# kr-colab/locator

Hardware: AMD Instinct MI355X
Metric: training samples/sec on 1000x100k-SNP matrix (higher is better)
Workload: dtype f32; 1 GPU; synthetic 1000 ind x 100000 SNPs uint8 (BASELINE.json configs[2]), single model fit per GPU, batch 32, 810 train / 90 validation; width=256, nlayers=10, graph=True, chained_steps=True, epochs_in_flight=2, replicates_per_gpu=1, replicates=single model, full=False

## Files before the change

locator_amd/csrc/stack_fused.hip:

```cpp
#include <stdlib.h>

#include <type_traits>

#include "common.h"
#include "stack_tail.h"

#ifndef SF_THREADS
#define SF_THREADS 512
#endif


__device__ __forceinline__ float sf_sumsq_train(float e0, float e1) {
#pragma clang fp contract(off)
    const float a = e0 * e0, b = e1 * e1;
    return b + a;
}
__device__ __forceinline__ float sf_sumsq_eval(float e0, float e1) { return fmaf(e1, e1, e0 * e0); }

template <int NHT, int R, bool TRAIN>
__global__ __launch_bounds__(SF_THREADS) void stack_fused_kernel(
    const float* __restrict__ a1_in, const float* __restrict__ Wh, const float* __restrict__ WhT,
    const float* __restrict__ bh, const float* __restrict__ wa, const float* __restrict__ ba,
    const float* __restrict__ wb, const float* __restrict__ bb, const uint8_t* __restrict__ mask, float keep_scale,
    int L, int n_pre, int n_b, const int32_t* __restrict__ rows, const float* __restrict__ Y,
    float* __restrict__ acts, float* __restrict__ adrop, float* __restrict__ dz, float* __restrict__ head_out,
    float* __restrict__ yhat, float* __restrict__ dist, int xcd_stride, int n_work, int slot_rows,
    const float* __restrict__ rd_partial, int rd_G, int64_t rd_MH, const float* __restrict__ rd_cvec8,
    const float* __restrict__ rd_b1) {
    constexpr int Hp = NHT * 32;
    constexpr int C4 = Hp / 4;
    constexpr int KG = SF_THREADS / C4;
    constexpr int KPG = Hp / KG;
    static_assert(SF_THREADS % C4 == 0 && Hp % KG == 0 && KPG >= 1, "unsupported width for the fused stack");
    __shared__ __attribute__((aligned(16))) float act[R][Hp];
    __shared__ __attribute__((aligned(16))) float part[KG][R][Hp];
    __shared__ float hs[R][8];

    if (xcd_stride > 1 && (blockIdx.x % xcd_stride) != 0) return;
    const int li = xcd_stride > 1 ? blockIdx.x / xcd_stride : blockIdx.x;
    if (li >= n_work) {
        const int n_x = xcd_stride > 1 ? 8 / xcd_stride : 1;
        const int nh_all = (int)(gridDim.x / (xcd_stride > 1 ? xcd_stride : 1)) - n_work;
        const int hid = (li - n_work) / n_x, nh = nh_all / n_x > 0 ? nh_all / n_x : 1;
        const int64_t n4 = (int64_t)(L - 1) * Hp * Hp / 4;
        const f32x4* w4 = reinterpret_cast<const f32x4*>(Wh);
        f32x4 sink = {0.f, 0.f, 0.f, 0.f};
        for (int64_t i = (int64_t)hid * SF_THREADS + threadIdx.x; i < n4; i += (int64_t)nh * SF_THREADS) {
            f32x4 v = w4[i];
            sink[0] += v[0];
        }
        if (TRAIN && WhT != nullptr) {
            const f32x4* t4 = reinterpret_cast<const f32x4*>(WhT);
            for (int64_t i = n4 - 1 - ((int64_t)hid * SF_THREADS + threadIdx.x); i >= 0; i -= (int64_t)nh * SF_THREADS) {
                f32x4 v = t4[i];
                sink[1] += v[0];
            }
        }
        asm volatile("" ::"v"(sink[0]), "v"(sink[1]));
        return;
    }
    const int t = threadIdx.x, c4 = t % C4, kq = t / C4;
    const int r0 = li * R;
    const int64_t blk = (int64_t)slot_rows * Hp, HH = (int64_t)Hp * Hp;

    constexpr int RING = KPG < 32 ? KPG : 32;
    constexpr int RW = RING >= 16 ? RING / 8 : 1;
    constexpr int NS = RING / RW, NTRIP = KPG / RING;
    constexpr int ROWB = C4 * 16;
    static_assert(KPG >= 2 && NS >= 2 && NS * RW == RING && NTRIP * RING == KPG, "a pass must be whole trips round the ring");
    static_assert(ROWB <= 4096 && (RW == 1 || 4096 % ROWB == 0), "row offsets are split into a register part and an immediate");
    constexpr int NO = (R * Hp + SF_THREADS - 1) / SF_THREADS;
    static_assert((R * Hp) % SF_THREADS == 0 || R * Hp < SF_THREADS, "epilogue slots");
    f32x4 ring[RING];
    constexpr int NOFF = (RW * ROWB + 4095) / 4096;
    uint32_t toff[NOFF];
#pragma unroll
    for (int n = 0; n < NOFF; ++n) toff[n] = ((uint32_t)(kq * KPG) * C4 + c4) * 16u + 4096u * n;
    auto load_slot = [&](const float* __restrict__ Wsrc, int c, int s) {
        const char* base = reinterpret_cast<const char*>(Wsrc) + (size_t)c * (RW * ROWB);
        static_assert(RW == 1 || RW == 4, "rows per slot");
        gload16_uniform<0>(ring[s * RW], base, toff[0]);
        if constexpr (RW == 4) {
            gload16_uniform<ROWB % 4096>(ring[s * RW + 1], base, toff[ROWB / 4096]);
            gload16_uniform<(2 * ROWB) % 4096>(ring[s * RW + 2], base, toff[2 * ROWB / 4096]);
            gload16_uniform<(3 * ROWB) % 4096>(ring[s * RW + 3], base, toff[3 * ROWB / 4096]);
        }
    };
    auto fma_slot = [&](int c, int s, f32x4 (&acc)[R]) {
#pragma unroll
        for (int j = 0; j < RW; ++j) {
#pragma unroll
            for (int r = 0; r < R; ++r) {
                const float a = act[r][kq * KPG + c * RW + j];
                acc[r][0] = fmaf(a, ring[s * RW + j][0], acc[r][0]);
                acc[r][1] = fmaf(a, ring[s * RW + j][1], acc[r][1]);
                acc[r][2] = fmaf(a, ring[s * RW + j][2], acc[r][2]);
                acc[r][3] = fmaf(a, ring[s * RW + j][3], acc[r][3]);
            }
        }
    };
    auto trip = [&](auto last, int c0, const float* __restrict__ Wn, int cn, f32x4 (&acc)[R]) {
        constexpr int N = (NS - 1) * RW + (decltype(last)::value ? NO : 0);
#pragma unroll
        for (int s = 0; s < NS; ++s) {
            if constexpr (RW == 4) vm_wait_slot<N>(ring[s * RW], ring[s * RW + 1], ring[s * RW + 2], ring[s * RW + 3]);
            else vm_wait_slot<N>(ring[s * RW]);
            fma_slot(c0 + s, s, acc);
#pragma unroll
            for (int r = 0; r < R; ++r) vm_landed(acc[r]);
            load_slot(Wn, cn + s, s);
        }
    };
    auto contract = [&](const float* __restrict__ Wcur, const float* __restrict__ Wnext, auto operands) {
        f32x4 acc[R];
#pragma unroll
        for (int r = 0; r < R; ++r) acc[r] = f32x4{0.f, 0.f, 0.f, 0.f};
#pragma unroll 1
        for (int tr = 0; tr + 1 < NTRIP; ++tr) trip(std::false_type{}, tr * NS, Wcur, (tr + 1) * NS, acc);
        operands();
        trip(std::true_type{}, (NTRIP - 1) * NS, Wnext, 0, acc);
#pragma unroll
        for (int r = 0; r < R; ++r) *reinterpret_cast<f32x4*>(&part[kq][r][4 * c4]) = acc[r];
    };
    auto ring_end = [&]() {
        vm_wait<0>();
#pragma unroll
        for (int k = 0; k < RING; ++k) vm_landed(ring[k]);
    };
    const int n_pass = TRAIN ? 2 * (L - 1) : (L - 1);
    auto wseq = [&](int p) -> const float* {
        if (p >= n_pass) return uniform_ptr(Wh);
        return uniform_ptr(p < L - 1 ? Wh + (int64_t)p * HH : WhT + (int64_t)(2 * (L - 1) - 1 - p) * HH);
    };
    auto ring_start = [&]() {
        const float* W0 = wseq(0);
#pragma unroll
        for (int s = 0; s < NS; ++s) load_slot(W0, s, s);
    };
    auto reduced = [&](int r, int n) {
        float s = 0.f;
#pragma unroll
        for (int g = 0; g < KG; ++g) s += part[g][r][n];
        return s;
    };

    static_assert(SF_THREADS % Hp == 0, "one pair of wa per thread needs a thread count that is a multiple of the width");
    float h_wa0 = 0.f, h_wa1 = 0.f;
    float h_ba0 = 0.f, h_ba1 = 0.f, h_w00 = 0.f, h_w01 = 0.f, h_w10 = 0.f, h_w11 = 0.f, h_bb0 = 0.f, h_bb1 = 0.f;
    float h_y0 = 0.f, h_y1 = 0.f;
    const bool has_y = Y != nullptr && t < R && r0 + t < n_b;

    if (!TRAIN && rd_partial != nullptr) {
        const int gq = (rd_G + 3) / 4;
        for (int i = t; i < R * Hp; i += SF_THREADS) {
            const int r = i / Hp, n = i % Hp;
            float v = 0.f;
            if (r0 + r < n_b) {
                const float* src = rd_partial + (int64_t)(r0 + r) * Hp + n;
                float sq[4];
#pragma unroll
                for (int q = 0; q < 4; ++q) {
                    const int g0 = q * gq, g1 = g0 + gq < rd_G ? g0 + gq : rd_G;
                    float z = 0.f;
                    for (int g = g0; g < g1; ++g) z += src[(int64_t)g * rd_MH];
                    sq[q] = z;
                }
                float c = rd_cvec8[n];
#pragma unroll
                for (int sl = 1; sl < 8; ++sl) c += rd_cvec8[sl * Hp + n];
                v = elu_f((((sq[0] + sq[1]) + sq[2]) + sq[3]) + (c + rd_b1[n]));
            }
            act[r][n] = v;
        }
    }
    {
        const bool stage = TRAIN || rd_partial == nullptr;
        float a1v[NO];
        uint32_t yrow = 0;
#pragma unroll
        for (int o = 0; o < NO; ++o) {
            const int i = t + SF_THREADS * o;
            a1v[o] = 0.f;
            if (stage && i < R * Hp) gload4_inout(a1v[o], a1_in + (int64_t)(r0 + i / Hp) * Hp + i % Hp);
        }
        if (has_y) gload4_inout(yrow, rows + r0 + t);
        gload4_inout(h_wa0, wa + 2 * (t % Hp));
        gload4_inout(h_wa1, wa + 2 * (t % Hp) + 1);
        if (t < R) {
            gload4_inout(h_ba0, ba); gload4_inout(h_ba1, ba + 1);
            gload4_inout(h_w00, wb); gload4_inout(h_w01, wb + 1); gload4_inout(h_w10, wb + 2); gload4_inout(h_w11, wb + 3);
            gload4_inout(h_bb0, bb); gload4_inout(h_bb1, bb + 1);
        }
        ring_start();
        vm_wait<RING>();
#pragma unroll
        for (int o = 0; o < NO; ++o) vm_landed(a1v[o]);
        vm_landed(yrow);
        vm_landed(h_wa0); vm_landed(h_wa1);
        vm_landed(h_ba0); vm_landed(h_ba1); vm_landed(h_w00); vm_landed(h_w01); vm_landed(h_w10); vm_landed(h_w11);
        vm_landed(h_bb0); vm_landed(h_bb1);
        if (has_y) { gload4_inout(h_y0, Y + (int64_t)(int32_t)yrow * 2); gload4_inout(h_y1, Y + (int64_t)(int32_t)yrow * 2 + 1); }
#pragma unroll
        for (int o = 0; o < NO; ++o) {
            const int i = t + SF_THREADS * o;
            if (stage && i < R * Hp) act[i / Hp][i % Hp] = a1v[o];
        }
    }
    lds_barrier();

    for (int l = 2; l <= L; ++l) {
        const float* bias = bh + (int64_t)(l - 2) * Hp;
        const bool dr = TRAIN && mask != nullptr && l == n_pre;
        float e_bias[NO];
        uint32_t e_m[NO];
        contract(wseq(l - 2), wseq(l - 1), [&]() {
#pragma unroll
            for (int o = 0; o < NO; ++o) {
                const int i = (t + SF_THREADS * o) % (R * Hp);
                e_bias[o] = 0.f;
                gload4_inout(e_bias[o], bias + i % Hp);
                e_m[o] = 1;
                if (dr) gload1_inout(e_m[o], mask + (int64_t)(r0 + i / Hp) * Hp + i % Hp);
            }
        });
        lds_barrier();
        vm_wait<RING>();
#pragma unroll
        for (int o = 0; o < NO; ++o) { vm_landed(e_bias[o]); vm_landed(e_m[o]); }
        vm_landed(h_y0); vm_landed(h_y1);
        float* aout = acts + (int64_t)(l - 1) * blk;
#pragma unroll
        for (int o = 0; o < NO; ++o) {
            const int i = t + SF_THREADS * o;
            if (i < R * Hp) {
                const int r = i / Hp, n = i % Hp;
                const float a = elu_f(reduced(r, n) + e_bias[o]);
                const int64_t gi = (int64_t)(r0 + r) * Hp + n;
                if (TRAIN) aout[gi] = a;
                float nx = a;
                if (dr) {
                    nx = a * (e_m[o] ? keep_scale : 0.f);
                    adrop[gi] = nx;
                }
                act[r][n] = nx;
            }
        }
        lds_barrier();
    }

    {
        float p0[R], p1[R];
#pragma unroll
        for (int r = 0; r < R; ++r) { p0[r] = 0.f; p1[r] = 0.f; }
        if (t < Hp) {
#pragma unroll
            for (int r = 0; r < R; ++r) { p0[r] = act[r][t] * h_wa0; p1[r] = act[r][t] * h_wa1; }
        }
#pragma unroll
        for (int r = 0; r < R; ++r) {
#pragma unroll
            for (int o = 1; o < 64; o <<= 1) { p0[r] += __shfl_xor(p0[r], o); p1[r] += __shfl_xor(p1[r], o); }
            if ((t & 63) == 0) { part[0][r][2 * (t >> 6)] = p0[r]; part[0][r][2 * (t >> 6) + 1] = p1[r]; }
        }
        lds_barrier();
        if (t < R) {
            const int r = t, b = r0 + r;
            float y10 = h_ba0, y11 = h_ba1;
            for (int w = 0; w < SF_THREADS / 64; ++w) { y10 += part[0][r][2 * w]; y11 += part[0][r][2 * w + 1]; }
            const float w00 = h_w00, w01 = h_w01, w10 = h_w10, w11 = h_w11;
            const float y20 = y10 * w00 + y11 * w10 + h_bb0;
            const float y21 = y10 * w01 + y11 * w11 + h_bb1;
            float d = 0.f, g0 = 0.f, g1 = 0.f;
            const bool valid = b < n_b;
            if (valid && Y != nullptr) {
                const float e0 = y20 - h_y0, e1 = y21 - h_y1;
                d = sqrtf(fmaxf(TRAIN ? sf_sumsq_train(e0, e1) : sf_sumsq_eval(e0, e1), 0.f));
                if (d > 0.f) { g0 = e0 / d / (float)n_b; g1 = e1 / d / (float)n_b; }
            }
            if (TRAIN) {
                const float dy10 = g0 * w00 + g1 * w01, dy11 = g0 * w10 + g1 * w11;
                hs[r][0] = dy10; hs[r][1] = dy11;
                float* ho = head_out + 8 * b;
                ho[0] = d; ho[1] = dy10; ho[2] = dy11; ho[3] = y10; ho[4] = y11; ho[5] = g0; ho[6] = g1; ho[7] = 0.f;
            } else if (valid) {
                yhat[2 * b] = y20; yhat[2 * b + 1] = y21;
                if (dist) dist[b] = d;
            }
        }
        lds_barrier();
    }
    if (!TRAIN) {
        ring_end();
        return;
    }

    {
        float* dzo = dz + (int64_t)(L - 1) * blk;
#pragma unroll
        for (int o = 0; o < NO; ++o) {
            const int i = t + SF_THREADS * o;
            if (i < R * Hp) {
                const int r = i / Hp, k = i % Hp;
                const float v = (hs[r][0] * h_wa0 + hs[r][1] * h_wa1) * elu_grad_from_act(act[r][k]);
                dzo[(int64_t)(r0 + r) * Hp + k] = v;
                part[0][r][k] = v;
            }
        }
        lds_barrier();
        for (int i = t; i < R * Hp; i += SF_THREADS) act[i / Hp][i % Hp] = part[0][i / Hp][i % Hp];
        lds_barrier();
    }
    for (int l = L; l >= 2; --l) {
        const int p = (L - 1) + (L - l);
        const float* aprev = acts + (int64_t)(l - 2) * blk;
        const bool dr = mask != nullptr && l - 1 == n_pre;
        float e_a[NO];
        uint32_t e_m[NO];
        contract(wseq(p), wseq(p + 1), [&]() {
#pragma unroll
            for (int o = 0; o < NO; ++o) {
                const int i = (t + SF_THREADS * o) % (R * Hp);
                const int64_t gi = (int64_t)(r0 + i / Hp) * Hp + i % Hp;
                e_a[o] = 0.f;
                gload4_inout(e_a[o], aprev + gi);
                e_m[o] = 1;
                if (dr) gload1_inout(e_m[o], mask + gi);
            }
        });
        lds_barrier();
        vm_wait<RING>();
#pragma unroll
        for (int o = 0; o < NO; ++o) { vm_landed(e_a[o]); vm_landed(e_m[o]); }
        float* dzo = dz + (int64_t)(l - 2) * blk;
#pragma unroll
        for (int o = 0; o < NO; ++o) {
            const int i = t + SF_THREADS * o;
            if (i < R * Hp) {
                const int r = i / Hp, k = i % Hp;
                float keep = 1.f;
                if (dr) keep = e_m[o] ? keep_scale : 0.f;
                const float v = reduced(r, k) * (keep * elu_grad_from_act(e_a[o]));
                dzo[(int64_t)(r0 + r) * Hp + k] = v;
                act[r][k] = v;
            }
        }
        lds_barrier();
    }
    ring_end();
}

template <int NHT, int RB>
__global__ __launch_bounds__(512) void stack_dw_all_kernel(loc_dw_tail_args ta, loc_gb_tail gb) {
    stack_dw_all_body<NHT, RB>((int)blockIdx.x, ta, gb);
}

__global__ void transpose_hidden_kernel(const float* __restrict__ Wh, float* __restrict__ WhT, int Hp, int nl) {
    __shared__ float tile[32][33];
    const int l = blockIdx.z, bx = blockIdx.x * 32, by = blockIdx.y * 32, tx = threadIdx.x & 31, ty = threadIdx.x >> 5;
    const float* src = Wh + (int64_t)l * Hp * Hp;
    float* dst = WhT + (int64_t)l * Hp * Hp;
    for (int j = ty; j < 32; j += 8) tile[j][tx] = src[(int64_t)(by + j) * Hp + bx + tx];
    __syncthreads();
    for (int j = ty; j < 32; j += 8) dst[(int64_t)(bx + j) * Hp + by + tx] = tile[tx][j];
    (void)nl;
}

extern "C" int loc_stack_fused_supported(int Hp) { return Hp == 64 || Hp == 128 || Hp == 256 || Hp == 512; }

#define SF_SWITCH(MACRO)                                                    \
    switch (Hp) {                                                           \
        case 64: MACRO(2); break;                                           \
        case 128: MACRO(4); break;                                          \
        case 256: MACRO(8); break;                                          \
        case 512: MACRO(16); break;                                         \
        default: loc_set_error("%s: fused stack needs width 64/128/256/512 after padding (got %d)", __func__, Hp); return -1; \
    }

extern "C" int loc_transpose_hidden(const float* Wh, float* WhT, int Hp, int n_hidden, void* stream) {
    if (n_hidden <= 0) return 0;
    hipLaunchKernelGGL(transpose_hidden_kernel, dim3(Hp / 32, Hp / 32, n_hidden), dim3(256), 0, (hipStream_t)stream, Wh,
                       WhT, Hp, n_hidden);
    LOC_CHECK_LAUNCH();
    return 0;
}

constexpr int SF_R = 2;
static int sf_train_rows(const loc_tuning* tune, int n_b) {
    const int v = tune ? tune->stack_train_rows : 0;
    (void)n_b;
    return (v == 1 || v == 2 || v == 4) ? v : 1;
}

static int sf_helpers(const loc_tuning* tune) {
    if (!tune || tune->stack_helpers == 0) return 12;
    return tune->stack_helpers < 0 ? 0 : tune->stack_helpers;
}
static int sf_xcd_stride(const loc_tuning* tune) {
    const int v = tune ? tune->stack_xcd_stride : 0;
    return v == 1 || v == 2 || v == 4 || v == 8 ? v : 8;
}

extern "C" int loc_stack_forward_backward(const float* a1_in, const float* Wh, const float* WhT, const float* bh,
                                          const float* wa, const float* ba, const float* wb, const float* bb,
                                          const uint8_t* mask, float keep_scale, int Hp, int L, int n_pre, int n_b,
                                          int slot_rows, const int32_t* rows, const float* Y, float* acts,
                                          float* adrop, float* dz, float* head_out, const loc_tuning* tune,
                                          void* stream) {
    if (n_b < 1 || n_b > slot_rows || slot_rows % 32 || L < 2) {
        loc_set_error("loc_stack_forward_backward: n_b=%d, slot_rows=%d, L=%d", n_b, slot_rows, L);
        return -1;
    }
    const int rpw = sf_train_rows(tune, n_b);
    const int nblk = (n_b + 31) / 32 * (32 / rpw);
    int xs = sf_xcd_stride(tune);
    int nh = xs > 1 ? sf_helpers(tune) : 0;
    while (xs > 1 && (nblk + nh + 8 / xs - 1) / (8 / xs) > 32) {
        xs /= 2;
        nh = (nh + 8 / xs - 1) / (8 / xs) * (8 / xs);
    }
    if (xs == 1) nh = 0;
#define LAUNCH_TR(N, RR)                                                                                           \
    hipLaunchKernelGGL((stack_fused_kernel<N, RR, true>), dim3((nblk + nh) * xs), dim3(SF_THREADS), 0,             \
                       (hipStream_t)stream, a1_in, Wh, WhT, bh, wa, ba, wb, bb, mask, keep_scale, L, n_pre, n_b,  \
                       rows, Y, acts, adrop, dz, head_out, (float*)nullptr, (float*)nullptr, xs, nblk, slot_rows,         \
                       (const float*)nullptr, 0, (int64_t)0, (const float*)nullptr, (const float*)nullptr);
#define LAUNCH1(N) LAUNCH_TR(N, 1)
#define LAUNCH2(N) LAUNCH_TR(N, 2)
#define LAUNCH4(N) LAUNCH_TR(N, 4)
    if (rpw == 1) { SF_SWITCH(LAUNCH1) } else if (rpw == 4) { SF_SWITCH(LAUNCH4) } else { SF_SWITCH(LAUNCH2) }
#undef LAUNCH1
#undef LAUNCH2
#undef LAUNCH4
#undef LAUNCH_TR
    LOC_CHECK_LAUNCH();
    return 0;
}

static int sf_eval_launch(const float* a1, const float* rd_partial, int rd_G, int64_t rd_MH, const float* rd_cvec8,
                          const float* rd_b1, const float* Wh, const float* bh, const float* wa, const float* ba,
                          const float* wb, const float* bb, int Hp, int L, int n_b, const int32_t* rows, const float* Y,
                          float* yhat, float* dist, void* stream, int rows_form = 0) {
    if (L < 2) {
        loc_set_error("hidden stack of a predict: L=%d (needs at least one hidden layer pass)", L);
        return -1;
    }
    if (rows_form >= 0 && loc_stack_rows_supported(Hp, L) && (rows_form > 0 || n_b >= loc_stack_rows_min_rows()))
        return sr_eval_launch(a1, rd_partial, rd_G, rd_MH, rd_cvec8, rd_b1, Wh, bh, wa, ba, wb, bb, L, n_b, rows, Y, yhat, dist,
                              rows_form == 1 ? 32 : rows_form == 2 ? 16 : 0, stream);
    const loc_tuning* tune = nullptr;
    int rpw = SF_R;
    if (Hp == 256) {
        const int cu = sr_compute_units();
        if (rows_form == -2 || (rows_form == 0 && n_b > 2 * cu && n_b <= 4 * cu)) rpw = 4;
        else if (rows_form == -3 || (rows_form == 0 && n_b > 4 * cu)) rpw = 8;
    }
    const int nblk = (n_b + rpw - 1) / rpw;
    int xs = sf_xcd_stride(tune);
    int nh = xs > 1 ? sf_helpers(tune) : 0;
    while (xs > 1 && (nblk + nh + 8 / xs - 1) / (8 / xs) > 32) {
        xs /= 2;
        nh = (nh + 8 / xs - 1) / (8 / xs) * (8 / xs);
    }
    if (xs == 1) nh = 0;
#define LAUNCH_R(N, RR)                                                                                           \
    hipLaunchKernelGGL((stack_fused_kernel<N, RR, false>), dim3((nblk + nh) * xs), dim3(SF_THREADS), 0,           \
                       (hipStream_t)stream, a1, Wh, (const float*)nullptr, bh, wa, ba, wb, bb,                    \
                       (const uint8_t*)nullptr, 1.f, L, 0, n_b, rows, Y, (float*)nullptr, (float*)nullptr,        \
                       (float*)nullptr, (float*)nullptr, yhat, dist, xs, nblk, 32, rd_partial, rd_G, rd_MH, rd_cvec8,  \
                       rd_b1);
#define LAUNCH(N) LAUNCH_R(N, SF_R)
    if (rpw == 4) { LAUNCH_R(8, 4) }
    else if (rpw == 8) { LAUNCH_R(8, 8) }

    else { SF_SWITCH(LAUNCH) }
#undef LAUNCH
#undef LAUNCH_R
    LOC_CHECK_LAUNCH();
    return 0;
}

extern "C" int loc_stack_forward_eval(const float* a1, const float* Wh, const float* bh, const float* wa,
                                      const float* ba, const float* wb, const float* bb, int Hp, int L, int n_b,
                                      const int32_t* rows, const float* Y, float* yhat, float* dist, void* stream) {
    return sf_eval_launch(a1, nullptr, 0, 0, nullptr, nullptr, Wh, bh, wa, ba, wb, bb, Hp, L, n_b, rows, Y, yhat, dist, stream);
}
extern "C" int loc_stack_forward_eval_form(const float* a1, const float* Wh, const float* bh, const float* wa,
                                           const float* ba, const float* wb, const float* bb, int Hp, int L, int n_b,
                                           const int32_t* rows, const float* Y, float* yhat, float* dist, int rows_form,
                                           void* stream) {
    return sf_eval_launch(a1, nullptr, 0, 0, nullptr, nullptr, Wh, bh, wa, ba, wb, bb, Hp, L, n_b, rows, Y, yhat, dist, stream,
                          rows_form);
}

extern "C" int loc_stack_forward_eval_partial(const float* partial, int groups, int64_t group_stride, const float* cvec8,
                                              const float* b1, const float* Wh, const float* bh, const float* wa,
                                              const float* ba, const float* wb, const float* bb, int Hp, int L, int n_b,
                                              const int32_t* rows, const float* Y, float* yhat, float* dist, int rows_form,
                                              void* stream) {
    if (!partial || groups < 1 || group_stride < (int64_t)n_b * Hp || !cvec8 || !b1) {
        loc_set_error("loc_stack_forward_eval_partial: groups=%d group_stride=%lld n_b=%d", groups, (long long)group_stride, n_b);
        return -1;
    }
    return sf_eval_launch(nullptr, partial, groups, group_stride, cvec8, b1, Wh, bh, wa, ba, wb, bb, Hp, L, n_b, rows, Y, yhat,
                          dist, stream, rows_form);
}

extern "C" int loc_stack_dw_adam_tail(int Hp, int L, int n_pre, int n_b, int slot_rows, int use_drop, const float* acts,
                                      const float* adrop, const float* dz, const float* head_out, float* params,
                                      float* adam_m, float* adam_v, float* WhT, int64_t off_wh, int64_t off_bh,
                                      int64_t off_wa, int64_t off_ba, int64_t off_wb, int64_t off_bb,
                                      float* loss_out, const float* alpha_tab, int alpha_tab_len, const float* lr,
                                      const int* t_base, int t_off, const loc_gb_tail* gb, void* stream) {
    if (n_b < 1 || n_b > LOC_BIG_BATCH_MAX || n_b > slot_rows) {
        loc_set_error("loc_stack_dw_adam: n_b=%d (limit %d), slot_rows=%d", n_b, LOC_BIG_BATCH_MAX, slot_rows);
        return -1;
    }
    const int nht = Hp / 32;
    loc_gb_tail g;
    if (gb) g = *gb; else { g = loc_gb_tail{}; g.K = 0; }
    const int grid = (L - 1) * nht * nht + 1 + (g.K > 0 ? (g.K + 511) / 512 : 0);
    loc_dw_tail_args ta;
    ta.L = L; ta.n_pre = n_pre; ta.n_b = n_b; ta.use_drop = use_drop;
    ta.acts = acts; ta.adrop = adrop; ta.dz = dz; ta.head_out = head_out;
    ta.P = params; ta.M = adam_m; ta.V = adam_v; ta.WhT = WhT;
    ta.off_wh = off_wh; ta.off_bh = off_bh; ta.off_wa = off_wa; ta.off_ba = off_ba; ta.off_wb = off_wb; ta.off_bb = off_bb;
    ta.loss_out = loss_out; ta.alpha_tab = alpha_tab; ta.alpha_tab_len = alpha_tab_len; ta.lr = lr; ta.t_base = t_base;
    ta.t_off = t_off; ta.slot_rows = slot_rows;
#define LAUNCH_RB(N, R) \
    hipLaunchKernelGGL((stack_dw_all_kernel<N, R>), dim3(grid), dim3(512), 0, (hipStream_t)stream, ta, g);
#define LAUNCH(N)                                                                                                 \
    switch ((n_b + 31) / 32) {                                                                                    \
        case 1: LAUNCH_RB(N, 1) break;                                                                            \
        case 2: LAUNCH_RB(N, 2) break;                                                                            \
        case 3: LAUNCH_RB(N, 3) break;                                                                            \
        case 4: LAUNCH_RB(N, 4) break;                                                                            \
        default: LAUNCH_RB(N, 0) break;                             \
    }
    SF_SWITCH(LAUNCH)
#undef LAUNCH
#undef LAUNCH_RB
    LOC_CHECK_LAUNCH();
    return 0;
}

extern "C" int loc_stack_dw_adam(int Hp, int L, int n_pre, int n_b, int use_drop, const float* acts,
                                 const float* adrop, const float* dz, const float* head_out, float* params,
                                 float* adam_m, float* adam_v, float* WhT, int64_t off_wh, int64_t off_bh,
                                 int64_t off_wa, int64_t off_ba, int64_t off_wb, int64_t off_bb, float* loss_out,
                                 const float* alpha_tab, int alpha_tab_len, const float* lr, const int* t_base,
                                 int t_off, void* stream) {
    return loc_stack_dw_adam_tail(Hp, L, n_pre, n_b, 32, use_drop, acts, adrop, dz, head_out, params, adam_m, adam_v, WhT,
                                  off_wh, off_bh, off_wa, off_ba, off_wb, off_bb, loss_out, alpha_tab, alpha_tab_len,
                                  lr, t_base, t_off, nullptr, stream);
}
```

Baseline: 194,900 samples/s.

## Prefetch leading weight slots of the pass after next into a head buffer

Adds a small register buffer (head) that holds the first HS ring slots of the weight matrix two passes ahead, loaded one pass early. At each layer turn those registers are copied into the ring, so the first slots of the next contraction need no fresh global load and the latency at the start of each pass is hidden. This costs extra VGPRs and changes the vmcnt wait accounting. It is only enabled by default for width 256 (NHT==8) with a single trip per pass.

```diff
diff --git a/locator_amd/csrc/stack_fused.hip b/locator_amd/csrc/stack_fused.hip
--- a/locator_amd/csrc/stack_fused.hip
+++ b/locator_amd/csrc/stack_fused.hip
@@ -16,6 +16,20 @@
     return b + a;
 }
 __device__ __forceinline__ float sf_sumsq_eval(float e0, float e1) { return fmaf(e1, e1, e0 * e0); }
+
+constexpr int sf_head_slots(int nht, int r, bool train) {
+    (void)r; (void)train;
+#ifdef SF_HEAD
+    (void)nht;
+    return SF_HEAD;
+#else
+    return nht == 8 ? 1 : 0;
+#endif
+}
+__device__ __forceinline__ void sf_head_to_ring(f32x4& ring, const f32x4& head) {
+    ring = head;
+    asm volatile("" : "+v"(ring) : "v"(head));
+}
 
 template <int NHT, int R, bool TRAIN>
 __global__ __launch_bounds__(SF_THREADS) void stack_fused_kernel(
@@ -72,6 +86,10 @@
     constexpr int NO = (R * Hp + SF_THREADS - 1) / SF_THREADS;
     static_assert((R * Hp) % SF_THREADS == 0 || R * Hp < SF_THREADS, "epilogue slots");
     f32x4 ring[RING];
+    constexpr int HS = NTRIP == 1 ? (sf_head_slots(NHT, R, TRAIN) < NS - 1 ? sf_head_slots(NHT, R, TRAIN) : NS - 1) : 0;
+    constexpr int HR = HS * RW;
+    static_assert(HS >= 0 && HS < NS, "slots HS .. NS-1 are the ones a pass requests again");
+    f32x4 head[HR > 0 ? HR : 1];
     constexpr int NOFF = (RW * ROWB + 4095) / 4096;
     uint32_t toff[NOFF];
 #pragma unroll
@@ -86,6 +104,18 @@
             gload16_uniform<(3 * ROWB) % 4096>(ring[s * RW + 3], base, toff[3 * ROWB / 4096]);
         }
     };
+    auto load_head = [&](const float* __restrict__ Wsrc) {
+#pragma unroll
+        for (int c = 0; c < HS; ++c) {
+            const char* base = reinterpret_cast<const char*>(Wsrc) + (size_t)c * (RW * ROWB);
+            gload16_uniform<0>(head[c * RW], base, toff[0]);
+            if constexpr (RW == 4) {
+                gload16_uniform<ROWB % 4096>(head[c * RW + 1], base, toff[ROWB / 4096]);
+                gload16_uniform<(2 * ROWB) % 4096>(head[c * RW + 2], base, toff[2 * ROWB / 4096]);
+                gload16_uniform<(3 * ROWB) % 4096>(head[c * RW + 3], base, toff[3 * ROWB / 4096]);
+            }
+        }
+    };
     auto fma_slot = [&](int c, int s, f32x4 (&acc)[R]) {
 #pragma unroll
         for (int j = 0; j < RW; ++j) {
@@ -101,14 +131,28 @@
     };
     auto trip = [&](auto last, int c0, const float* __restrict__ Wn, int cn, f32x4 (&acc)[R]) {
         constexpr int N = (NS - 1) * RW + (decltype(last)::value ? NO : 0);
+        auto wait_slot = [&](auto n, int s) {
+            if constexpr (RW == 4) vm_wait_slot<decltype(n)::value>(ring[s * RW], ring[s * RW + 1], ring[s * RW + 2], ring[s * RW + 3]);
+            else vm_wait_slot<decltype(n)::value>(ring[s * RW]);
+        };
 #pragma unroll
         for (int s = 0; s < NS; ++s) {
-            if constexpr (RW == 4) vm_wait_slot<N>(ring[s * RW], ring[s * RW + 1], ring[s * RW + 2], ring[s * RW + 3]);
-            else vm_wait_slot<N>(ring[s * RW]);
+            if (s < HS) wait_slot(std::integral_constant<int, RING + NO>{}, s);
+            else wait_slot(std::integral_constant<int, N>{}, s);
             fma_slot(c0 + s, s, acc);
 #pragma unroll
             for (int r = 0; r < R; ++r) vm_landed(acc[r]);
-            load_slot(Wn, cn + s, s);
+            if (s >= HS) load_slot(Wn, cn + s, s);
+        }
+    };
+    auto head_turn = [&](const float* __restrict__ Wnn) {
+        vm_wait<(NS - HS) * RW>();
+        if constexpr (HS > 0) {
+#pragma unroll
+            for (int k = 0; k < HR; ++k) vm_landed(head[k]);
+#pragma unroll
+            for (int k = 0; k < HR; ++k) sf_head_to_ring(ring[k], head[k]);
+            load_head(Wnn);
         }
     };
     auto contract = [&](const float* __restrict__ Wcur, const float* __restrict__ Wnext, auto operands) {
@@ -126,6 +170,8 @@
         vm_wait<0>();
 #pragma unroll
         for (int k = 0; k < RING; ++k) vm_landed(ring[k]);
+#pragma unroll
+        for (int k = 0; k < HR; ++k) vm_landed(head[k]);
     };
     const int n_pass = TRAIN ? 2 * (L - 1) : (L - 1);
     auto wseq = [&](int p) -> const float* {
@@ -136,6 +182,7 @@
         const float* W0 = wseq(0);
 #pragma unroll
         for (int s = 0; s < NS; ++s) load_slot(W0, s, s);
+        if constexpr (HS > 0) load_head(wseq(1));
     };
     auto reduced = [&](int r, int n) {
         float s = 0.f;
@@ -192,7 +239,7 @@
             gload4_inout(h_bb0, bb); gload4_inout(h_bb1, bb + 1);
         }
         ring_start();
-        vm_wait<RING>();
+        vm_wait<RING + HR>();
 #pragma unroll
         for (int o = 0; o < NO; ++o) vm_landed(a1v[o]);
         vm_landed(yrow);
@@ -224,7 +271,7 @@
             }
         });
         lds_barrier();
-        vm_wait<RING>();
+        head_turn(wseq(l));
 #pragma unroll
         for (int o = 0; o < NO; ++o) { vm_landed(e_bias[o]); vm_landed(e_m[o]); }
         vm_landed(h_y0); vm_landed(h_y1);
@@ -328,7 +375,7 @@
             }
         });
         lds_barrier();
-        vm_wait<RING>();
+        head_turn(wseq(p + 2));
 #pragma unroll
         for (int o = 0; o < NO; ++o) { vm_landed(e_a[o]); vm_landed(e_m[o]); }
         float* dzo = dz + (int64_t)(l - 2) * blk;
```

Measured after the change: 196,400 samples/s, median of 6. About the same (+0.8%).
